# proroklab/graph-conv-memory

Hardware: AMD Instinct MI355X
Metric: belief-states/sec (BxT) DenseGCM fwd+bwd, graph_size=128 F=32 (higher is better)
Workload: dtype f32; 1 GPU; cfg2: DenseGCM + TemporalBackedge([1,2,4]), B=256/GPU, graph_size=128, obs=32, hidden=32, 2x DenseGraphConv+tanh, T=128; one bench step = one rollout through the per-step drop-in call surface `for t: mx, m = gcm(obs[t], m)` + backward; B_per_gpu=256, graph_size=128, obs=32, hidden=32, T=128, state=donated (DenseGCM(donate_state=True): hidden state advanced in place), parallelism=dp1 (batch-sharded, 1 flat-bucket all-reduce per backward)

## Files before the change

graph-conv-memory_amd/csrc/rows_cached_run.hip:

```cpp
#include <atomic>
#include <new>
#include <type_traits>

#include "fused_common.h"
#include "gcm_common.h"
#include "rows_common.h"
#include "rows_head.h"
#include "rows_lean.h"

namespace gcm_rows {

constexpr int RUN_CAP = GCM_ROWS_MAX_STEPS;
constexpr int RUN_WAVES = 8;
constexpr int RUN_PAIRS = RUN_CAP / 2 / RUN_WAVES;
constexpr int RUN_OCTS = RUN_CAP / 8 / RUN_WAVES;
constexpr int RUN_WSTAGE = 2 * 16 * 64 / (64 * RUN_WAVES);

struct RunTable {
  const float* obs[RUN_CAP];
  float* rec[RUN_CAP];
};

struct FreshArgs {
  HeadSrcs hs;
  float* packed;
  float* image;
  unsigned pad0, pad0_end, pad1, pad1_end;
};
struct NoFresh {};
constexpr int RUN_ADJ_TAB = 256 + 128;

#ifndef GCM_RUN_FRESH_STORES_LATE
#define GCM_RUN_FRESH_STORES_LATE 0
#endif

template <bool FRESH>
__global__ __launch_bounds__(64 * RUN_WAVES) void k_step_rows_cached_img4_lean_run(
    const float* __restrict__ image, float* __restrict__ nodes, float* __restrict__ cH, const float* __restrict__ params,
    int cur0_arg, int n, unsigned hops4, unsigned nhs, float* __restrict__ adj, int64_t* __restrict__ count,
    float* __restrict__ cA, float* __restrict__ cX, uint32_t* __restrict__ flags, unsigned o_v, unsigned o_hdr,
    unsigned o_coef, unsigned o_live, int rec, RunTable tab, std::conditional_t<FRESH, FreshArgs, NoFresh> fr) {
  constexpr int F = 32, H1 = 32, ROWS = 128 * 32;
  const int cur0 = FRESH ? 0 : cur0_arg;
  __shared__ __attribute__((aligned(16))) float sXH[2 * ROWS];
  __shared__ __attribute__((aligned(16))) float svw[RUN_WAVES * 128];
  __shared__ __attribute__((aligned(16))) f32x2 sW[2 * 16 * 32 * 2];
  __shared__ float sadj[FRESH ? RUN_ADJ_TAB : 1];
  const int lane = threadIdx.x & 63;
  const int wv = __builtin_amdgcn_readfirstlane((int)(threadIdx.x >> 6));
  const unsigned gb = blockIdx.x;
  const unsigned N = nhs & 0xffu;
  const int H2 = (int)((nhs >> 8) & 0xffu);
  const bool self = (nhs >> 16) & 1u;
  const unsigned g0 = gb * N;
  const int fl = lane & 31, hs = lane >> 5;
  float* sv = svw + 128 * wv + 64 * hs;
  const int ol = fl < H2 ? fl : H2 - 1;
  float* recd[RUN_OCTS];
#pragma unroll
  for (int j = 0; j < RUN_OCTS; ++j) {
    const int t = 8 * (wv + RUN_WAVES * j) + (lane >> 3);
    recd[j] = tab.rec[t < n ? t : n - 1];
  }
  float xo[RUN_PAIRS];
  float* recp[RUN_PAIRS];
#pragma unroll
  for (int j = 0; j < RUN_PAIRS; ++j) {
    const int t = 2 * (wv + RUN_WAVES * j) + hs;
    const int tc = t < n ? t : n - 1;
    xo[j] = tab.obs[tc][gb * F + fl];
    recp[j] = tab.rec[tc];
  }
  f32x2 wst[RUN_WSTAGE];
  f32x4 wq[2];
  float bias1, bias2;
  float v_img = 0.f, v_pack = 0.f;
  const size_t e_first = (size_t)gb + (size_t)gridDim.x * threadIdx.x, e_wave = (size_t)gb + (size_t)gridDim.x * (64 * wv);
  if constexpr (!FRESH) {
    const f32x2* i3 = reinterpret_cast<const f32x2*>(image + 2 * 4 * 64 * 64);
#pragma unroll
    for (int r = 0; r < RUN_WSTAGE; ++r) wst[r] = i3[(int)threadIdx.x + 64 * RUN_WAVES * r];
    const float* b1 = params + 2 * H1 * F;
    bias1 = b1[fl];
    bias2 = b1[H1 + 2 * H2 * H1 + ol];
  } else {
#pragma unroll
    for (int r = 0; r < 2; ++r) {
      const int q = (int)threadIdx.x + 64 * RUN_WAVES * r;
      const int m = q >> 8, h = (q >> 3) & 31;
      const float* w = m == 0 ? fr.hs.p[0] : m == 1 ? fr.hs.p[1] : m == 2 ? fr.hs.p[3] : fr.hs.p[4];
      wq[r] = f32x4{0.f, 0.f, 0.f, 0.f};
      if (m < 2 || h < H2) wq[r] = *reinterpret_cast<const f32x4*>(w + h * 32 + 4 * (q & 7));
    }
    bias1 = fr.hs.p[2][fl];
    bias2 = fr.hs.p[5][ol];
    if (e_wave < (size_t)IMG_LAYOUT_FLOATS && e_first < (size_t)IMG_LAYOUT_FLOATS) {
      const int e = (int)e_first;
      v_img = head_image_value(fr.hs, e >> 12, (e >> 6) & 63, e & 63, F, H1, H2);
    }
    if (e_wave < fr.hs.off[HEAD_MAX_SRCS] && e_first < fr.hs.off[HEAD_MAX_SRCS])
      v_pack = head_packed_value(fr.hs, (unsigned)e_first);
  }
  int hmax = 0, nh = 0;
#pragma unroll
  for (int i = 0; i < 4; ++i) {
    const int h = (int)((hops4 >> (8 * i)) & 0xffu);
    if (h != 0xff) {
      ++nh;
      if (h > hmax) hmax = h;
    }
  }
  {
    const int lo = cur0 - hmax > 0 ? cur0 - hmax : 0;
    const float* src = hs ? cH : nodes;
    for (int r = lo + wv; r < cur0; r += RUN_WAVES) sXH[hs * ROWS + r * 32 + fl] = src[(g0 + (unsigned)r) * 32 + fl];
  }
  if constexpr (!FRESH) {
#pragma unroll
    for (int r = 0; r < RUN_WSTAGE; ++r) {
      const int e = (int)threadIdx.x + 64 * RUN_WAVES * r;
      sW[image3_lds_pair(e)] = wst[r];
    }
  } else {
    float* sWf = reinterpret_cast<float*>(sW);
#pragma unroll
    for (int r = 0; r < 2; ++r) {
      const int q = (int)threadIdx.x + 64 * RUN_WAVES * r;
#pragma unroll
      for (int u = 0; u < 4; ++u) sWf[image3_lds_index(q >> 8, 4 * (q & 7) + u, (q >> 3) & 31)] = wq[r][u];
    }
    if (threadIdx.x < RUN_ADJ_TAB) {
      const int d = 128 - (int)threadIdx.x;
      bool hit = d == 0 && self;
#pragma unroll
      for (int i = 0; i < 4; ++i) hit = hit || (d > 0 && (int)((hops4 >> (8 * i)) & 0xffu) == d);
      sadj[threadIdx.x] = hit && threadIdx.x < 256 ? 1.f : 0.f;
    }
  }
#pragma unroll
  for (int j = 0; j < RUN_PAIRS; ++j) {
    const int t = 2 * (wv + RUN_WAVES * j) + hs;
    if (t < n) {
      sXH[(cur0 + t) * 32 + fl] = xo[j];
      const unsigned at = (g0 + (unsigned)(cur0 + t)) * F + fl;
      nodes[at] = xo[j];
      cX[at] = xo[j];
    }
  }
  __syncthreads();
  auto fresh_stores = [&]() {
    if constexpr (FRESH) {
      const f32x4 z = {0.f, 0.f, 0.f, 0.f};
      const int nq = (int)(N >> 2);
      f32x4* arow = reinterpret_cast<f32x4*>(adj + (size_t)g0 * N);
      for (int r = 2 * wv + hs; r < (int)N; r += 2 * RUN_WAVES) {
        if (fl < nq) {
          const float* at = sadj + (r < n ? 128 + 4 * fl - r : 256);
          arow[r * nq + fl] = f32x4{at[0], at[1], at[2], at[3]};
        }
      }
      f32x4* nrow = reinterpret_cast<f32x4*>(nodes + (size_t)g0 * F);
      for (int i = n * (F / 4) + (int)threadIdx.x; i < (int)N * (F / 4); i += 64 * RUN_WAVES) nrow[i] = z;
      if (gb == 0 && threadIdx.x < 64) {
        if (fr.pad0 + threadIdx.x < fr.pad0_end) nodes[fr.pad0 + threadIdx.x] = 0.f;
        if (fr.pad1 + threadIdx.x < fr.pad1_end) nodes[fr.pad1 + threadIdx.x] = 0.f;
      }
      if (e_wave < (size_t)IMG_LAYOUT_FLOATS && e_first < (size_t)IMG_LAYOUT_FLOATS) head_image_store(fr.image, (int)e_first, v_img);
      if (e_wave < fr.hs.off[HEAD_MAX_SRCS] && e_first < fr.hs.off[HEAD_MAX_SRCS]) fr.packed[e_first] = v_pack;
    }
  };
  if (!GCM_RUN_FRESH_STORES_LATE) fresh_stores();
  auto sources = [&](int cur, const float* rows, float (&va)[4]) {
    int k = 0;
#pragma unroll
    for (int i = 0; i < 4; ++i) k += (int)(((hops4 >> (8 * i)) & 0xffu) <= (unsigned)cur);
#pragma unroll
    for (int q = 0; q < 4; ++q) {
      const int idx = k - 1 - q;
      const bool any = idx >= 0;
      const int s = any ? cur - (int)((hops4 >> (8 * (idx & 3))) & 0xffu) : 0;
      const float v = rows[s * 32 + fl];
      va[q] = any ? v : 0.f;
    }
  };
  int back[4];
  bool has[4];
#pragma unroll
  for (int q = 0; q < 4; ++q) {
    const int idx = nh - 1 - q;
    has[q] = idx >= 0;
    back[q] = has[q] ? 32 * (int)((hops4 >> (8 * (idx & 3))) & 0xffu) : 0;
  }
  auto sources_all = [&](int cur, const float* rows, float (&va)[4]) {
    const float* at = rows + cur * 32 + fl;
#pragma unroll
    for (int q = 0; q < 4; ++q) {
      const float v = *(at - back[q]);
      va[q] = has[q] ? v : 0.f;
    }
  };
  f32x2 wa[16], wb[16];
  auto weights = [&](int layer) {
#pragma unroll
    for (int k = 0; k < 16; ++k) {
      const f32x4 q = *reinterpret_cast<const f32x4*>(sW + ((layer * 16 + k) * 32 + fl) * 2);
      wa[k] = f32x2{q[0], q[1]};
      wb[k] = f32x2{q[2], q[3]};
    }
  };
  auto matvec = [&]() { return lean_half_chain(wa, sv, 0) + lean_half_chain(wb, sv, 1); };
  weights(0);
  auto layer1 = [&](int cur, bool live, const float (&xa)[4]) {
    const unsigned rc = g0 + (unsigned)cur;
    const float xc = sXH[cur * 32 + fl];
    asm volatile("" ::: "memory");
    float agg1 = (xa[0] + xa[1]) + (xa[2] + xa[3]);
    agg1 = agg1 + (self ? xc : 0.f);
    *reinterpret_cast<f32x2*>(sv + 2 * fl) = f32x2{agg1, xc};
    asm volatile("" ::: "memory");
    const float p1 = bias1 + matvec();
    const float h1c = gcm_tanh(p1);
    asm volatile("" ::: "memory");
    if (live) {
      sXH[ROWS + cur * 32 + fl] = h1c;
      cA[rc * F + fl] = agg1;
      cH[rc * H1 + fl] = h1c;
    }
  };
#pragma unroll
  for (int j = 0; j < RUN_PAIRS; ++j) {
    const int t0 = 2 * (wv + RUN_WAVES * j);
    if (t0 >= n) break;
    const bool live = t0 + hs < n;
    const int cur = cur0 + (live ? t0 + hs : n - 1);
    float xa[4];
    if (cur0 + t0 < hmax) sources(cur, sXH, xa);
    else sources_all(cur, sXH, xa);
    layer1(cur, live, xa);
  }
  __syncthreads();
  weights(1);
  bool bad = false;
  auto layer2 = [&](int cur, bool live, float* saved, const float (&ha)[4]) {
    const float h1c = sXH[ROWS + cur * 32 + fl];
    asm volatile("" ::: "memory");
    float agg2 = (ha[0] + ha[1]) + (ha[2] + ha[3]);
    agg2 = agg2 + (self ? h1c : 0.f);
    *reinterpret_cast<f32x2*>(sv + 2 * fl) = f32x2{agg2, h1c};
    asm volatile("" ::: "memory");
    const float p2 = bias2 + matvec();
    const float v = gcm_tanh(p2);
    asm volatile("" ::: "memory");
    if (live && fl < H2) saved[gb * H2 + fl] = v;
    if (rec && live) {
      saved[o_v + gb * 2 * H1 + fl] = agg2;
      saved[o_v + gb * 2 * H1 + H1 + fl] = h1c;
    }
    bad = bad || (live && fl < H2 && !isfinite(v));
  };
#pragma unroll
  for (int j = 0; j < RUN_PAIRS; ++j) {
    const int t0 = 2 * (wv + RUN_WAVES * j);
    if (t0 >= n) break;
    const bool live = t0 + hs < n;
    const int cur = cur0 + (live ? t0 + hs : n - 1);
    float ha[4];
    if (cur0 + t0 < hmax) sources(cur, sXH + ROWS, ha);
    else sources_all(cur, sXH + ROWS, ha);
    layer2(cur, live, recp[j], ha);
  }
#pragma unroll
  for (int o = 0; o < RUN_OCTS; ++o) {
    const int t = 8 * (wv + RUN_WAVES * o) + (lane >> 3);
    if (t < n) {
      const int q = lane & 7;
      const int cur = cur0 + t;
      int k = 0;
#pragma unroll
      for (int i = 0; i < 4; ++i) k += (int)(((hops4 >> (8 * i)) & 0xffu) <= (unsigned)cur);
      const int j = q < k ? cur - (int)((hops4 >> (8 * ((k - 1 - q) & 3))) & 0xffu) : cur;
      const bool is_cur = q == k;
      if (!FRESH && (q < k || (is_cur && self))) adj[(size_t)(g0 + (unsigned)cur) * N + j] = 1.f;
      if (rec) {
        float* saved = recd[o];
        if (q <= k) {
          (reinterpret_cast<int*>(saved + o_live) + gb * N)[q] = j;
          (saved + o_coef + gb * N)[q] = (is_cur && !self) ? 0.f : 1.f;
        }
        if (q == 7) {
          int* hdr = reinterpret_cast<int*>(saved + o_hdr) + 4 * gb;
          hdr[0] = k + 1; hdr[1] = k; hdr[2] = cur; hdr[3] = 0;
        }
      }
    }
  }
  if (threadIdx.x == 0) count[gb] = cur0 + n;
  const bool nonfinite = __any(bad);
  if (nonfinite && lane == 0) atomicOr(flags, GCM_FLAG_NONFINITE);
  if constexpr (FRESH) {
    if (GCM_RUN_FRESH_STORES_LATE) fresh_stores();
    const size_t step = (size_t)gridDim.x * (64 * RUN_WAVES);
    for (size_t e = e_first + step; e < (size_t)IMG_LAYOUT_FLOATS; e += step)
      head_image_store(fr.image, (int)e, head_image_value(fr.hs, (int)e >> 12, ((int)e >> 6) & 63, (int)e & 63, F, H1, H2));
    for (size_t e = e_first + step; e < fr.hs.off[HEAD_MAX_SRCS]; e += step) fr.packed[e] = head_packed_value(fr.hs, (unsigned)e);
  }
}

struct Run {
  hipGraphNode_t node = nullptr;
  unsigned long long cid = 0;
  hipStream_t stream = nullptr;
  int n = 0, cur0 = 0;
  float *nodes = nullptr, *adj = nullptr, *cH = nullptr, *cA = nullptr, *cX = nullptr;
  int64_t* count = nullptr;
  const float *params = nullptr, *image = nullptr;
  uint32_t* flags = nullptr;
  int B = 0, N = 0, H2 = 0, self = 0, rec = 0;
  unsigned hops4 = 0xffffffffu;
  RunTable tab;
  int cap = RUN_CAP;
  unsigned long long stat_cid = 0;
  int stat_nodes = 0, stat_merged = 0, stat_absorbed = 0;
  struct Head {
    hipGraphNode_t node = nullptr;
    unsigned long long cid = 0;
    hipStream_t stream = nullptr;
    HeadSrcs hs{};
    float *packed = nullptr, *image = nullptr;
    void* zero = nullptr;
    size_t zero_bytes = 0;
    int H2 = 0;
  } head;
  bool absorb = true, fresh = false;
  FreshArgs fr{};
};

static std::atomic<bool> g_merge_ok{true};
static std::atomic<int> g_route{0}, g_last_error{0};

static void merge_off(hipError_t e) {
  g_last_error = (int)e;
  g_merge_ok = false;
  (void)hipGetLastError();
}
static std::atomic<bool> g_absorb_ok{true};
static void absorb_off(hipError_t e) {
  g_last_error = (int)e;
  g_absorb_ok = false;
  (void)hipGetLastError();
}

struct RunArgs {
  int cur0, n, rec;
  unsigned hops4, nhs, o_v, o_hdr, o_coef, o_live;
  NoFresh none;
  void* ptr[20];
  hipKernelNodeParams p;
};
static void fill_args(Run& R, int n, RunArgs& a) {
  const CachedLayout lay = make_cached_layout(R.B, R.N, 32, R.H2);
  a.cur0 = R.cur0;
  a.n = n;
  a.rec = R.rec;
  a.hops4 = R.hops4;
  a.nhs = (unsigned)R.N | (unsigned)R.H2 << 8 | (R.self ? 1u << 16 : 0u);
  a.o_v = (unsigned)lay.o_v; a.o_hdr = (unsigned)lay.o_hdr; a.o_coef = (unsigned)lay.o_coef; a.o_live = (unsigned)lay.o_live;
  void* ptr[20] = {&R.image, &R.nodes, &R.cH, &R.params, &a.cur0, &a.n, &a.hops4, &a.nhs, &R.adj, &R.count,
                   &R.cA,    &R.cX,    &R.flags, &a.o_v, &a.o_hdr, &a.o_coef, &a.o_live, &a.rec, &R.tab,
                   R.fresh ? (void*)&R.fr : (void*)&a.none};
  for (int i = 0; i < 20; ++i) a.ptr[i] = ptr[i];
  a.p = hipKernelNodeParams{};
  a.p.func = R.fresh ? (void*)k_step_rows_cached_img4_lean_run<true> : (void*)k_step_rows_cached_img4_lean_run<false>;
  a.p.gridDim = dim3(R.B);
  a.p.blockDim = dim3(64 * RUN_WAVES);
  a.p.sharedMemBytes = 0;
  a.p.kernelParams = a.ptr;
  a.p.extra = nullptr;
}

inline int64_t pad64(int64_t v) { return (v + 63) & ~int64_t(63); }

static int absorb_head(Run& R, int n, hipGraph_t graph, hipError_t* broken) {
  const Run::Head& H = R.head;
  if (!R.absorb || !g_absorb_ok.load() || R.fresh || R.cur0 != 0 || !H.node || H.cid != R.cid || H.stream != R.stream)
    return 0;
  const int64_t n_nodes = pad64((int64_t)R.B * R.N * 32), n_adj = pad64((int64_t)R.B * R.N * R.N);
  const auto aligned16 = [](const void* p) { return (reinterpret_cast<uintptr_t>(p) & 15) == 0; };
  if (H.packed != R.params || H.image != R.image || H.H2 != R.H2 || R.N % 4 != 0 || H.zero != (void*)R.nodes ||
      H.zero_bytes != sizeof(float) * (size_t)(n_nodes + n_adj + 2 * (int64_t)R.B) || R.adj != R.nodes + n_nodes ||
      reinterpret_cast<float*>(R.count) != R.nodes + n_nodes + n_adj || !aligned16(H.hs.p[0]) || !aligned16(H.hs.p[1]) ||
      !aligned16(H.hs.p[3]) || !aligned16(H.hs.p[4]))
    return 0;
  size_t nd = 0, n_dep = 0, nh = 0;
  hipGraphNode_t one = nullptr, hdeps[8];
  hipError_t e = hipGraphNodeGetDependentNodes(R.node, nullptr, &n_dep);
  if (e == hipSuccess && n_dep) return 0;
  if (e == hipSuccess) e = hipGraphNodeGetDependencies(R.node, nullptr, &nd);
  if (e == hipSuccess && nd != 1) return 0;
  if (e == hipSuccess) e = hipGraphNodeGetDependencies(R.node, &one, &nd);
  if (e == hipSuccess && (nd != 1 || one != H.node)) return 0;
  if (e == hipSuccess) e = hipGraphNodeGetDependentNodes(H.node, nullptr, &n_dep);
  if (e == hipSuccess && n_dep != 1) return 0;
  if (e == hipSuccess) e = hipGraphNodeGetDependentNodes(H.node, &one, &n_dep);
  if (e == hipSuccess && (n_dep != 1 || one != R.node)) return 0;
  if (e == hipSuccess) e = hipGraphNodeGetDependencies(H.node, nullptr, &nh);
  if (e == hipSuccess && nh > 8) return 0;
  if (e == hipSuccess && nh) e = hipGraphNodeGetDependencies(H.node, hdeps, &nh);
  if (e != hipSuccess) {
    absorb_off(e);
    return 0;
  }
  R.fr = FreshArgs{};
  R.fr.hs = H.hs;
  R.fr.packed = H.packed;
  R.fr.image = H.image;
  R.fr.pad0 = (unsigned)((int64_t)R.B * R.N * 32);
  R.fr.pad0_end = (unsigned)n_nodes;
  R.fr.pad1 = (unsigned)(n_nodes + (int64_t)R.B * R.N * R.N);
  R.fr.pad1_end = (unsigned)(n_nodes + n_adj);
  R.fresh = true;
  RunArgs a;
  fill_args(R, n, a);
  hipGraphNode_t fresh = nullptr;
  e = hipGraphAddKernelNode(&fresh, graph, nh ? hdeps : nullptr, nh, &a.p);
  if (e != hipSuccess) {
    R.fresh = false;
    absorb_off(e);
    return 0;
  }
  e = hipStreamUpdateCaptureDependencies(R.stream, &fresh, 1, hipStreamSetCaptureDependencies);
  if (e == hipSuccess) {
    e = hipGraphDestroyNode(R.node);
    if (e != hipSuccess) {
      hipGraphNode_t old = R.node;
      (void)hipStreamUpdateCaptureDependencies(R.stream, &old, 1, hipStreamSetCaptureDependencies);
    }
  }
  if (e != hipSuccess) {
    (void)hipGraphDestroyNode(fresh);
    R.fresh = false;
    absorb_off(e);
    return 0;
  }
  R.node = fresh;
  g_route = 2;
  e = hipGraphDestroyNode(H.node);
  if (e != hipSuccess) {
    absorb_off(e);
    hipGraphNode_t from = H.node;
    const hipError_t e2 = hipGraphAddDependencies(graph, &from, &fresh, 1);
    if (e2 != hipSuccess) {
      (void)hipGetLastError();
      *broken = e;
      R.node = nullptr;
      R.head.node = nullptr;
      return 0;
    }
  } else {
    ++R.stat_absorbed;
  }
  R.head.node = nullptr;
  return 1;
}

static bool grow_node(Run& R, int n, hipGraph_t graph, hipError_t* broken) {
  if (R.n == 1 && n == 2) {
    const int ab = absorb_head(R, n, graph, broken);
    if (ab || *broken != hipSuccess) return ab == 1;
  }
  RunArgs a;
  fill_args(R, n, a);
  if (g_route.load() != 2) {
    const hipError_t e = hipGraphKernelNodeSetParams(R.node, &a.p);
    if (e == hipSuccess) {
      g_route = 1;
      return true;
    }
    g_last_error = (int)e;
    (void)hipGetLastError();
    if (g_route.load() == 1) {
      merge_off(e);
      return false;
    }
  }
  size_t nd = 0, n_dependent = 0;
  hipError_t e = hipGraphNodeGetDependentNodes(R.node, nullptr, &n_dependent);
  if (e == hipSuccess && n_dependent) return false;
  if (e == hipSuccess) e = hipGraphNodeGetDependencies(R.node, nullptr, &nd);
  hipGraphNode_t deps[8];
  if (e == hipSuccess && nd > 8) e = hipErrorInvalidValue;
  if (e == hipSuccess && nd) e = hipGraphNodeGetDependencies(R.node, deps, &nd);
  hipGraphNode_t fresh = nullptr;
  if (e == hipSuccess) e = hipGraphAddKernelNode(&fresh, graph, nd ? deps : nullptr, nd, &a.p);
  if (e != hipSuccess) {
    merge_off(e);
    return false;
  }
  e = hipStreamUpdateCaptureDependencies(R.stream, &fresh, 1, hipStreamSetCaptureDependencies);
  if (e != hipSuccess) {
    (void)hipGraphDestroyNode(fresh);
    merge_off(e);
    return false;
  }
  e = hipGraphDestroyNode(R.node);
  if (e != hipSuccess) {
    hipGraphNode_t old = R.node;
    (void)hipStreamUpdateCaptureDependencies(R.stream, &old, 1, hipStreamSetCaptureDependencies);
    (void)hipGraphDestroyNode(fresh);
    merge_off(e);
    return false;
  }
  R.node = fresh;
  g_route = 2;
  return true;
}

static bool overlap(const float* p, size_t floats, const float* q, size_t floats2) {
  return p < q + floats2 && q < p + floats;
}

static bool shares_memory(const Run& R, const float* obs, const float* saved, size_t obs_floats, size_t rec_floats) {
  for (int t = 0; t < R.n; ++t)
    if (overlap(saved, rec_floats, R.tab.rec[t], rec_floats) || overlap(saved, rec_floats, R.tab.obs[t], obs_floats) ||
        overlap(obs, obs_floats, R.tab.rec[t], rec_floats))
      return true;
  return false;
}

}

extern "C" int gcm_rows_run_steps_cap(void) { return gcm_rows::RUN_CAP; }
extern "C" void* gcm_rows_run_create(void) { return new (std::nothrow) gcm_rows::Run(); }
extern "C" int gcm_rows_run_destroy(void* run) {
  delete static_cast<gcm_rows::Run*>(run);
  return GCM_OK;
}
extern "C" int gcm_rows_run_reset(void* run) {
  GCM_REQUIRE(run);
  static_cast<gcm_rows::Run*>(run)->node = nullptr;
  static_cast<gcm_rows::Run*>(run)->fresh = false;
  return GCM_OK;
}
extern "C" int gcm_rows_run_set_cap(void* run, int cap) {
  GCM_REQUIRE(run && cap >= 1 && cap <= gcm_rows::RUN_CAP);
  static_cast<gcm_rows::Run*>(run)->cap = cap;
  return GCM_OK;
}
extern "C" int gcm_rows_run_stats(const void* run, int* out2) {
  GCM_REQUIRE(run && out2);
  const gcm_rows::Run* R = static_cast<const gcm_rows::Run*>(run);
  out2[0] = R->stat_nodes;
  out2[1] = R->stat_merged;
  return GCM_OK;
}
extern "C" int gcm_rows_run_enabled(void) { return gcm_rows::g_merge_ok.load() ? 1 : 0; }
extern "C" int gcm_rows_run_route(int* out2) {
  GCM_REQUIRE(out2);
  out2[0] = gcm_rows::g_route.load();
  out2[1] = gcm_rows::g_last_error.load();
  return GCM_OK;
}

extern "C" int gcm_dense_rows_step_cached_run(void* run, const float* obs, float* nodes, float* adj, int64_t* count,
                                              const gcm_selector_desc* selectors, int n_selectors, const float* params,
                                              const float* weight_image, int has_bias, int act1, int act2,
                                              float* cache_h1, float* cache_agg1, float* cache_nodes, float* saved,
                                              int record, int cur_host, uint32_t* flags, void* workspace,
                                              size_t workspace_bytes, int B, int N, int F, int H1, int H2,
                                              gcm_stream_t stream) {
  using namespace gcm_rows;
  auto plain = [&]() {
    return gcm_dense_rows_step_cached_ws(obs, nodes, adj, count, selectors, n_selectors, params, weight_image, has_bias,
                                         act1, act2, cache_h1, cache_agg1, cache_nodes, saved, record, cur_host, flags,
                                         workspace, workspace_bytes, B, N, F, H1, H2, stream);
  };
  Run* R = static_cast<Run*>(run);
  if (!R || !g_merge_ok.load()) return plain();
  hipStream_t st = (hipStream_t)stream;
  hipStreamCaptureStatus cs = hipStreamCaptureStatusNone;
  unsigned long long cid = 0;
  hipGraph_t graph = nullptr;
  const hipGraphNode_t* deps = nullptr;
  size_t nd = 0;
  hipError_t e = hipStreamGetCaptureInfo_v2(st, &cs, &cid, &graph, &deps, &nd);
  if (e != hipSuccess) {
    merge_off(e);
    return plain();
  }
  if (cs != hipStreamCaptureStatusActive) {
    R->node = nullptr;
    R->head.node = nullptr;
    R->fresh = false;
    R->stat_cid = 0;
    R->stat_nodes = R->stat_merged = R->stat_absorbed = 0;
    return plain();
  }
  GCM_REQUIRE(obs && nodes && adj && count && params && cache_h1 && cache_agg1 && cache_nodes && saved && flags);
  GCM_REQUIRE(B > 0 && (selectors || n_selectors == 0));
  LeanCase lc;
  CachedLayout lay = make_cached_layout(B, N, H1, H2);
  const bool lean = gcm_dense_rows_cached_supported_ws(selectors, n_selectors, has_bias, N, F, H1, H2) &&
                    (size_t)B * N * (size_t)(F > N ? F : N) < ((size_t)1 << 31) && lay.total < ((size_t)1 << 31) &&
                    lean_step_case(selectors, n_selectors, weight_image, has_bias, act1, act2, N, F, H1, H2, cur_host, lc);
  if (!lean) {
    R->node = nullptr;
    R->fresh = false;
    return plain();
  }
  const int self = lc.self;
  unsigned hops4 = 0xffffffffu;
  for (int a = 0; a < lc.nh; ++a) hops4 = (hops4 & ~(0xffu << (8 * a))) | (unsigned)lc.hops[a] << (8 * a);
  const size_t obs_floats = (size_t)B * F, rec_floats = record ? lay.total : (size_t)B * H2;
  const size_t rows_floats = (size_t)B * N * 32;
  const bool obs_in_state = overlap(obs, obs_floats, nodes, rows_floats) || overlap(obs, obs_floats, cache_nodes, rows_floats) ||
                            overlap(obs, obs_floats, cache_h1, rows_floats) || overlap(obs, obs_floats, cache_agg1, rows_floats) ||
                            overlap(obs, obs_floats, adj, (size_t)B * N * N);
  if (R->stat_cid != cid) {
    R->stat_cid = cid;
    R->stat_nodes = R->stat_merged = R->stat_absorbed = 0;
  }
  const bool follows = R->node && R->cid == cid && R->stream == st && nd == 1 && deps[0] == R->node &&
                       cur_host == R->cur0 + R->n && R->n < R->cap && R->n < RUN_CAP && R->nodes == nodes &&
                       R->adj == adj && R->count == count && R->cH == cache_h1 && R->cA == cache_agg1 &&
                       R->cX == cache_nodes && R->params == params && R->image == weight_image && R->flags == flags &&
                       R->B == B && R->N == N && R->H2 == H2 && R->self == self && R->hops4 == hops4 &&
                       R->rec == (record ? 1 : 0) && !obs_in_state &&
                       !shares_memory(*R, obs, saved, obs_floats, rec_floats);
  if (follows) {
    R->tab.obs[R->n] = obs;
    R->tab.rec[R->n] = saved;
    hipError_t broken = hipSuccess;
    if (grow_node(*R, R->n + 1, graph, &broken)) {
      ++R->n;
      ++R->stat_merged;
      return GCM_OK;
    }
    if (broken != hipSuccess) return (int)broken;
  }
  R->node = nullptr;
  R->fresh = false;
  if (!record) lay.total = 0;
  const int rc = launch_step_cached_lean(obs, nodes, adj, count, lc.m0, lc.m1, self, params, weight_image, cache_h1,
                                         cache_agg1, cache_nodes, saved, lay, flags, B, N, H2, cur_host, st);
  if (rc == GCM_EUNSUPPORTED) return plain();
  if (rc) return rc;
  ++R->stat_nodes;
  if (!g_merge_ok.load()) return GCM_OK;
  unsigned long long cid2 = 0;
  e = hipStreamGetCaptureInfo_v2(st, &cs, &cid2, &graph, &deps, &nd);
  if (e != hipSuccess) {
    merge_off(e);
    return GCM_OK;
  }
  if (cs != hipStreamCaptureStatusActive || cid2 != cid || nd != 1) return GCM_OK;
  hipGraphNode_t node = deps[0];
  hipGraphNodeType type;
  hipKernelNodeParams got;
  if ((e = hipGraphNodeGetType(node, &type)) != hipSuccess ||
      (type == hipGraphNodeTypeKernel && (e = hipGraphKernelNodeGetParams(node, &got)) != hipSuccess)) {
    merge_off(e);
    return GCM_OK;
  }
  if (type != hipGraphNodeTypeKernel || got.func != lean_step_kernel()) return GCM_OK;
  R->node = node;
  R->cid = cid;
  R->stream = st;
  R->n = 1;
  R->cur0 = cur_host;
  R->nodes = nodes; R->adj = adj; R->count = count; R->cH = cache_h1; R->cA = cache_agg1; R->cX = cache_nodes;
  R->params = params; R->image = weight_image; R->flags = flags;
  R->B = B; R->N = N; R->H2 = H2; R->self = self; R->rec = record ? 1 : 0;
  R->hops4 = hops4;
  R->tab.obs[0] = obs;
  R->tab.rec[0] = saved;
  return GCM_OK;
}

extern "C" int gcm_rows_run_set_absorb(void* run, int on) {
  GCM_REQUIRE(run);
  static_cast<gcm_rows::Run*>(run)->absorb = on != 0;
  return GCM_OK;
}
extern "C" int gcm_rows_run_absorbed(const void* run) {
  return run ? static_cast<const gcm_rows::Run*>(run)->stat_absorbed : 0;
}
extern "C" int gcm_rows_run_absorb_enabled(void) { return gcm_rows::g_absorb_ok.load() ? 1 : 0; }

extern "C" int gcm_dense_rows_head_fused_run(void* run, const float* const* srcs_host, const size_t* lens_host, int n,
                                             float* packed, float* image, int F, int H1, int H2, void* zero,
                                             size_t zero_bytes, gcm_stream_t stream) {
  using namespace gcm_rows;
  const int rc = gcm_dense_rows_head_fused(srcs_host, lens_host, n, packed, image, F, H1, H2, zero, zero_bytes, stream);
  Run* R = static_cast<Run*>(run);
  if (!R) return rc;
  R->head.node = nullptr;
  if (rc != GCM_OK || !R->absorb || !g_absorb_ok.load() || !g_merge_ok.load() || !image || !zero || F != 32 || H1 != 32)
    return rc;
  hipStream_t st = (hipStream_t)stream;
  hipStreamCaptureStatus cs = hipStreamCaptureStatusNone;
  unsigned long long cid = 0;
  hipGraph_t graph = nullptr;
  const hipGraphNode_t* deps = nullptr;
  size_t nd = 0;
  hipError_t e = hipStreamGetCaptureInfo_v2(st, &cs, &cid, &graph, &deps, &nd);
  if (e != hipSuccess) {
    absorb_off(e);
    return rc;
  }
  if (cs != hipStreamCaptureStatusActive || nd != 1) return rc;
  hipGraphNode_t node = deps[0];
  hipGraphNodeType type;
  hipKernelNodeParams got;
  if ((e = hipGraphNodeGetType(node, &type)) != hipSuccess ||
      (type == hipGraphNodeTypeKernel && (e = hipGraphKernelNodeGetParams(node, &got)) != hipSuccess)) {
    absorb_off(e);
    return rc;
  }
  if (type != hipGraphNodeTypeKernel || got.func != head_fused_kernel()) return rc;
  size_t total = 0;
  if (!head_make_srcs(srcs_host, lens_host, n, R->head.hs, total)) return rc;
  R->head.node = node;
  R->head.cid = cid;
  R->head.stream = st;
  R->head.packed = packed;
  R->head.image = image;
  R->head.zero = zero;
  R->head.zero_bytes = zero_bytes;
  R->head.H2 = H2;
  return rc;
}

extern "C" int gcm_rows_capture_node_count(gcm_stream_t stream) {
  hipStreamCaptureStatus cs = hipStreamCaptureStatusNone;
  unsigned long long cid = 0;
  hipGraph_t graph = nullptr;
  const hipGraphNode_t* deps = nullptr;
  size_t nd = 0, nodes = 0;
  if (hipStreamGetCaptureInfo_v2((hipStream_t)stream, &cs, &cid, &graph, &deps, &nd) != hipSuccess ||
      cs != hipStreamCaptureStatusActive || hipGraphGetNodes(graph, nullptr, &nodes) != hipSuccess) {
    (void)hipGetLastError();
    return -1;
  }
  return (int)nodes;
}
```

Measured before the change: 555.5 million belief-states/s.

## Precompute per-layer graph aggregates into LDS before matvec phases

The graph aggregation for each layer now runs as a separate phase. Threads compute it with vectorized f32x4 reads at precomputed source offsets and write the interleaved (agg, own) rows into a new LDS buffer sized for all steps. The matvec loops then read straight from that buffer, so per-wave scratch staging and per-step source lookups disappear. cA and record stores become vectorized when alignment allows. In exchange, LDS moves to dynamic allocation and grows considerably, and two extra block barriers are added, which may reduce occupancy.

```diff
diff --git a/graph-conv-memory_amd/csrc/rows_cached_run.hip b/graph-conv-memory_amd/csrc/rows_cached_run.hip
--- a/graph-conv-memory_amd/csrc/rows_cached_run.hip
+++ b/graph-conv-memory_amd/csrc/rows_cached_run.hip
@@ -15,6 +15,7 @@
 constexpr int RUN_PAIRS = RUN_CAP / 2 / RUN_WAVES;
 constexpr int RUN_OCTS = RUN_CAP / 8 / RUN_WAVES;
 constexpr int RUN_WSTAGE = 2 * 16 * 64 / (64 * RUN_WAVES);
+constexpr int RUN_AGG = RUN_CAP * 8 / (64 * RUN_WAVES);
 
 struct RunTable {
   const float* obs[RUN_CAP];
@@ -30,6 +31,11 @@
 struct NoFresh {};
 constexpr int RUN_ADJ_TAB = 256 + 128;
 
+constexpr int RUN_LDS_ROWS = 128 * 32, RUN_LDS_AX = 2 * RUN_LDS_ROWS, RUN_LDS_W = RUN_LDS_AX + RUN_CAP * 64,
+              RUN_LDS_ADJ = RUN_LDS_W + 2 * (2 * 16 * 32 * 2);
+constexpr size_t run_lds_bytes(bool fresh) { return sizeof(float) * (size_t)(RUN_LDS_ADJ + (fresh ? RUN_ADJ_TAB : 0)); }
+constexpr unsigned RUN_WIDE_ROWS = 1u << 17, RUN_WIDE_REC = 1u << 18;
+
 #ifndef GCM_RUN_FRESH_STORES_LATE
 #define GCM_RUN_FRESH_STORES_LATE 0
 #endif
@@ -42,10 +48,12 @@
     unsigned o_coef, unsigned o_live, int rec, RunTable tab, std::conditional_t<FRESH, FreshArgs, NoFresh> fr) {
   constexpr int F = 32, H1 = 32, ROWS = 128 * 32;
   const int cur0 = FRESH ? 0 : cur0_arg;
-  __shared__ __attribute__((aligned(16))) float sXH[2 * ROWS];
-  __shared__ __attribute__((aligned(16))) float svw[RUN_WAVES * 128];
-  __shared__ __attribute__((aligned(16))) f32x2 sW[2 * 16 * 32 * 2];
-  __shared__ float sadj[FRESH ? RUN_ADJ_TAB : 1];
+  static_assert(ROWS == RUN_LDS_ROWS, "the LDS layout");
+  extern __shared__ __attribute__((aligned(16))) float sRun[];
+  float* const sXH = sRun;
+  float* const sAX = sRun + RUN_LDS_AX;
+  f32x2* const sW = reinterpret_cast<f32x2*>(sRun + RUN_LDS_W);
+  float* const sadj = sRun + RUN_LDS_ADJ;
   const int lane = threadIdx.x & 63;
   const int wv = __builtin_amdgcn_readfirstlane((int)(threadIdx.x >> 6));
   const unsigned gb = blockIdx.x;
@@ -54,8 +62,10 @@
   const bool self = (nhs >> 16) & 1u;
   const unsigned g0 = gb * N;
   const int fl = lane & 31, hs = lane >> 5;
-  float* sv = svw + 128 * wv + 64 * hs;
+  const int ar = (int)(threadIdx.x >> 3), ac = (int)(threadIdx.x & 7);
+  const bool wide_rows = nhs & RUN_WIDE_ROWS, wide_rec = nhs & RUN_WIDE_REC;
   const int ol = fl < H2 ? fl : H2 - 1;
+  static_assert(RUN_AGG == RUN_OCTS, "the aggregate phases share phase D's record pointers");
   float* recd[RUN_OCTS];
 #pragma unroll
   for (int j = 0; j < RUN_OCTS; ++j) {
@@ -101,14 +111,11 @@
     if (e_wave < fr.hs.off[HEAD_MAX_SRCS] && e_first < fr.hs.off[HEAD_MAX_SRCS])
       v_pack = head_packed_value(fr.hs, (unsigned)e_first);
   }
-  int hmax = 0, nh = 0;
+  int hmax = 0;
 #pragma unroll
   for (int i = 0; i < 4; ++i) {
     const int h = (int)((hops4 >> (8 * i)) & 0xffu);
-    if (h != 0xff) {
-      ++nh;
-      if (h > hmax) hmax = h;
-    }
+    if (h != 0xff && h > hmax) hmax = h;
   }
   {
     const int lo = cur0 - hmax > 0 ? cur0 - hmax : 0;
@@ -136,6 +143,17 @@
       for (int i = 0; i < 4; ++i) hit = hit || (d > 0 && (int)((hops4 >> (8 * i)) & 0xffu) == d);
       sadj[threadIdx.x] = hit && threadIdx.x < 256 ? 1.f : 0.f;
     }
+  }
+  auto settle = [](auto v) { asm volatile("" ::"v"(v)); };
+#pragma unroll
+  for (int j = 0; j < RUN_OCTS; ++j) settle(recd[j]);
+#pragma unroll
+  for (int j = 0; j < RUN_PAIRS; ++j) settle(recp[j]);
+  settle(bias1);
+  settle(bias2);
+  if constexpr (FRESH) {
+    settle(v_img);
+    settle(v_pack);
   }
 #pragma unroll
   for (int j = 0; j < RUN_PAIRS; ++j) {
@@ -145,6 +163,23 @@
       const unsigned at = (g0 + (unsigned)(cur0 + t)) * F + fl;
       nodes[at] = xo[j];
       cX[at] = xo[j];
+    }
+  }
+  int soff[RUN_AGG][4];
+  unsigned sany = 0;
+#pragma unroll
+  for (int s = 0; s < RUN_AGG; ++s) {
+    const int cur = cur0 + ar + 64 * s;
+    int k = 0;
+#pragma unroll
+    for (int i = 0; i < 4; ++i) k += (int)(((hops4 >> (8 * i)) & 0xffu) <= (unsigned)cur);
+#pragma unroll
+    for (int q = 0; q < 4; ++q) {
+      const int idx = k - 1 - q;
+      const bool any = idx >= 0;
+      const int src = any ? cur - (int)((hops4 >> (8 * (idx & 3))) & 0xffu) : 0;
+      soff[s][q] = src * 32 + 4 * ac;
+      sany |= any ? 1u << (4 * s + q) : 0u;
     }
   }
   __syncthreads();
@@ -170,33 +205,35 @@
     }
   };
   if (!GCM_RUN_FRESH_STORES_LATE) fresh_stores();
-  auto sources = [&](int cur, const float* rows, float (&va)[4]) {
-    int k = 0;
-#pragma unroll
-    for (int i = 0; i < 4; ++i) k += (int)(((hops4 >> (8 * i)) & 0xffu) <= (unsigned)cur);
-#pragma unroll
-    for (int q = 0; q < 4; ++q) {
-      const int idx = k - 1 - q;
-      const bool any = idx >= 0;
-      const int s = any ? cur - (int)((hops4 >> (8 * (idx & 3))) & 0xffu) : 0;
-      const float v = rows[s * 32 + fl];
-      va[q] = any ? v : 0.f;
+  const f32x4 zero4 = {0.f, 0.f, 0.f, 0.f};
+  auto aggregate = [&](const float* rows, auto&& out) {
+#pragma unroll
+    for (int s = 0; s < RUN_AGG; ++s) {
+      const int t = ar + 64 * s;
+      if (t < n) {
+        const int cur = cur0 + t;
+        const f32x4 own = *reinterpret_cast<const f32x4*>(rows + cur * 32 + 4 * ac);
+        f32x4 v[4];
+#pragma unroll
+        for (int q = 0; q < 4; ++q) {
+          const f32x4 u = *reinterpret_cast<const f32x4*>(rows + soff[s][q]);
+          v[q] = (sany >> (4 * s + q)) & 1u ? u : zero4;
+        }
+        f32x4 agg = (v[0] + v[1]) + (v[2] + v[3]);
+        agg = agg + (self ? own : zero4);
+        f32x4* ax = reinterpret_cast<f32x4*>(sAX + t * 64 + 8 * ac);
+        ax[0] = f32x4{agg[0], own[0], agg[1], own[1]};
+        ax[1] = f32x4{agg[2], own[2], agg[3], own[3]};
+        out(s, cur, agg, own);
+      }
     }
   };
-  int back[4];
-  bool has[4];
-#pragma unroll
-  for (int q = 0; q < 4; ++q) {
-    const int idx = nh - 1 - q;
-    has[q] = idx >= 0;
-    back[q] = has[q] ? 32 * (int)((hops4 >> (8 * (idx & 3))) & 0xffu) : 0;
-  }
-  auto sources_all = [&](int cur, const float* rows, float (&va)[4]) {
-    const float* at = rows + cur * 32 + fl;
-#pragma unroll
-    for (int q = 0; q < 4; ++q) {
-      const float v = *(at - back[q]);
-      va[q] = has[q] ? v : 0.f;
+  auto store4 = [](float* at, const f32x4& v, bool wide) {
+    if (wide) {
+      *reinterpret_cast<f32x4*>(at) = v;
+    } else {
+#pragma unroll
+      for (int u = 0; u < 4; ++u) at[u] = v[u];
     }
   };
   f32x2 wa[16], wb[16];
@@ -208,66 +245,44 @@
       wb[k] = f32x2{q[2], q[3]};
     }
   };
-  auto matvec = [&]() { return lean_half_chain(wa, sv, 0) + lean_half_chain(wb, sv, 1); };
+  auto matvec = [&](const float* ax) { return lean_half_chain(wa, ax, 0) + lean_half_chain(wb, ax, 1); };
   weights(0);
-  auto layer1 = [&](int cur, bool live, const float (&xa)[4]) {
-    const unsigned rc = g0 + (unsigned)cur;
-    const float xc = sXH[cur * 32 + fl];
-    asm volatile("" ::: "memory");
-    float agg1 = (xa[0] + xa[1]) + (xa[2] + xa[3]);
-    agg1 = agg1 + (self ? xc : 0.f);
-    *reinterpret_cast<f32x2*>(sv + 2 * fl) = f32x2{agg1, xc};
-    asm volatile("" ::: "memory");
-    const float p1 = bias1 + matvec();
-    const float h1c = gcm_tanh(p1);
-    asm volatile("" ::: "memory");
-    if (live) {
-      sXH[ROWS + cur * 32 + fl] = h1c;
-      cA[rc * F + fl] = agg1;
-      cH[rc * H1 + fl] = h1c;
-    }
-  };
+  aggregate(sXH, [&](int, int cur, const f32x4& agg, const f32x4&) {
+    store4(cA + (g0 + (unsigned)cur) * F + 4 * ac, agg, wide_rows);
+  });
+  __syncthreads();
 #pragma unroll
   for (int j = 0; j < RUN_PAIRS; ++j) {
     const int t0 = 2 * (wv + RUN_WAVES * j);
     if (t0 >= n) break;
     const bool live = t0 + hs < n;
-    const int cur = cur0 + (live ? t0 + hs : n - 1);
-    float xa[4];
-    if (cur0 + t0 < hmax) sources(cur, sXH, xa);
-    else sources_all(cur, sXH, xa);
-    layer1(cur, live, xa);
+    const int t = live ? t0 + hs : n - 1;
+    const float h1c = gcm_tanh(bias1 + matvec(sAX + t * 64));
+    if (live) {
+      sXH[ROWS + (cur0 + t) * 32 + fl] = h1c;
+      cH[(g0 + (unsigned)(cur0 + t)) * H1 + fl] = h1c;
+    }
   }
   __syncthreads();
   weights(1);
+  aggregate(sXH + ROWS, [&](int s, int, const f32x4& agg, const f32x4& own) {
+    if (rec) {
+      float* at = recd[s] + o_v + gb * 2 * H1 + 4 * ac;
+      store4(at, agg, wide_rec);
+      store4(at + H1, own, wide_rec);
+    }
+  });
+  __syncthreads();
   bool bad = false;
-  auto layer2 = [&](int cur, bool live, float* saved, const float (&ha)[4]) {
-    const float h1c = sXH[ROWS + cur * 32 + fl];
-    asm volatile("" ::: "memory");
-    float agg2 = (ha[0] + ha[1]) + (ha[2] + ha[3]);
-    agg2 = agg2 + (self ? h1c : 0.f);
-    *reinterpret_cast<f32x2*>(sv + 2 * fl) = f32x2{agg2, h1c};
-    asm volatile("" ::: "memory");
-    const float p2 = bias2 + matvec();
-    const float v = gcm_tanh(p2);
-    asm volatile("" ::: "memory");
-    if (live && fl < H2) saved[gb * H2 + fl] = v;
-    if (rec && live) {
-      saved[o_v + gb * 2 * H1 + fl] = agg2;
-      saved[o_v + gb * 2 * H1 + H1 + fl] = h1c;
-    }
-    bad = bad || (live && fl < H2 && !isfinite(v));
-  };
 #pragma unroll
   for (int j = 0; j < RUN_PAIRS; ++j) {
     const int t0 = 2 * (wv + RUN_WAVES * j);
     if (t0 >= n) break;
     const bool live = t0 + hs < n;
-    const int cur = cur0 + (live ? t0 + hs : n - 1);
-    float ha[4];
-    if (cur0 + t0 < hmax) sources(cur, sXH + ROWS, ha);
-    else sources_all(cur, sXH + ROWS, ha);
-    layer2(cur, live, recp[j], ha);
+    const int t = live ? t0 + hs : n - 1;
+    const float v = gcm_tanh(bias2 + matvec(sAX + t * 64));
+    if (live && fl < H2) recp[j][gb * H2 + fl] = v;
+    bad = bad || (live && fl < H2 && !isfinite(v));
   }
 #pragma unroll
   for (int o = 0; o < RUN_OCTS; ++o) {
@@ -357,13 +372,18 @@
   void* ptr[20];
   hipKernelNodeParams p;
 };
+static bool aligned16(const void* p) { return (reinterpret_cast<uintptr_t>(p) & 15) == 0; }
 static void fill_args(Run& R, int n, RunArgs& a) {
   const CachedLayout lay = make_cached_layout(R.B, R.N, 32, R.H2);
+  const bool wide_rows = aligned16(R.cA);
+  bool wide_rec = lay.o_v % 4 == 0;
+  for (int t = 0; t < n; ++t) wide_rec = wide_rec && aligned16(R.tab.rec[t]);
   a.cur0 = R.cur0;
   a.n = n;
   a.rec = R.rec;
   a.hops4 = R.hops4;
-  a.nhs = (unsigned)R.N | (unsigned)R.H2 << 8 | (R.self ? 1u << 16 : 0u);
+  a.nhs = (unsigned)R.N | (unsigned)R.H2 << 8 | (R.self ? 1u << 16 : 0u) | (wide_rows ? RUN_WIDE_ROWS : 0u) |
+          (wide_rec ? RUN_WIDE_REC : 0u);
   a.o_v = (unsigned)lay.o_v; a.o_hdr = (unsigned)lay.o_hdr; a.o_coef = (unsigned)lay.o_coef; a.o_live = (unsigned)lay.o_live;
   void* ptr[20] = {&R.image, &R.nodes, &R.cH, &R.params, &a.cur0, &a.n, &a.hops4, &a.nhs, &R.adj, &R.count,
                    &R.cA,    &R.cX,    &R.flags, &a.o_v, &a.o_hdr, &a.o_coef, &a.o_live, &a.rec, &R.tab,
@@ -373,7 +393,8 @@
   a.p.func = R.fresh ? (void*)k_step_rows_cached_img4_lean_run<true> : (void*)k_step_rows_cached_img4_lean_run<false>;
   a.p.gridDim = dim3(R.B);
   a.p.blockDim = dim3(64 * RUN_WAVES);
-  a.p.sharedMemBytes = 0;
+  a.p.sharedMemBytes = (unsigned)run_lds_bytes(R.fresh);
+  gcm_allow_dynamic_lds(a.p.func, run_lds_bytes(R.fresh));
   a.p.kernelParams = a.ptr;
   a.p.extra = nullptr;
 }
@@ -385,7 +406,6 @@
   if (!R.absorb || !g_absorb_ok.load() || R.fresh || R.cur0 != 0 || !H.node || H.cid != R.cid || H.stream != R.stream)
     return 0;
   const int64_t n_nodes = pad64((int64_t)R.B * R.N * 32), n_adj = pad64((int64_t)R.B * R.N * R.N);
-  const auto aligned16 = [](const void* p) { return (reinterpret_cast<uintptr_t>(p) & 15) == 0; };
   if (H.packed != R.params || H.image != R.image || H.H2 != R.H2 || R.N % 4 != 0 || H.zero != (void*)R.nodes ||
       H.zero_bytes != sizeof(float) * (size_t)(n_nodes + n_adj + 2 * (int64_t)R.B) || R.adj != R.nodes + n_nodes ||
       reinterpret_cast<float*>(R.count) != R.nodes + n_nodes + n_adj || !aligned16(H.hs.p[0]) || !aligned16(H.hs.p[1]) ||
@@ -530,7 +550,11 @@
 }
 
 extern "C" int gcm_rows_run_steps_cap(void) { return gcm_rows::RUN_CAP; }
-extern "C" void* gcm_rows_run_create(void) { return new (std::nothrow) gcm_rows::Run(); }
+extern "C" void* gcm_rows_run_create(void) {
+  gcm_allow_dynamic_lds((const void*)gcm_rows::k_step_rows_cached_img4_lean_run<false>, gcm_rows::run_lds_bytes(false));
+  gcm_allow_dynamic_lds((const void*)gcm_rows::k_step_rows_cached_img4_lean_run<true>, gcm_rows::run_lds_bytes(true));
+  return new (std::nothrow) gcm_rows::Run();
+}
 extern "C" int gcm_rows_run_destroy(void* run) {
   delete static_cast<gcm_rows::Run*>(run);
   return GCM_OK;
```

Measured after the change: 560.6 million belief-states/s, median of 6. Within noise of the previous version (+0.9%).
